# facebookresearch/DLRM-FlexFlow

Measured on AMD Instinct MI355X. Metric: dlrm_training_samples_per_sec, higher is better.
Workload: dtype f32; 1 GPU; criteo-terabyte-shape: 26 tables (rows 39884406-39043-17289-7420-20263-3-7120-1543-63-38532951-2953546-403346-10-2208-11938-155-4-976-14-39979771-25641295-39664984-585935-12972-108-36), emb_dim 128, bag 1, bot 13-512-256-128, top 3456-1024-1024-512-256-1, cat interaction, SGD lr 0.01, MSE loss; global_batch=32768, per_gpu_batch=32768, parallelism=single GPU, hipGraph-replayed step, step_graph=True

## Files before the change

dlrm_flexflow_amd/host/ffmodel.h:

```cpp
#pragma once

#include <cstddef>
#include <cstdint>
#include <condition_variable>
#include <deque>
#include <functional>
#include <map>
#include <mutex>
#include <thread>
#include <string>
#include <vector>

#include "../../include/ff_hip.h"
#include "../../include/ff_hip_bf16.h"
#include "../../include/ff_hip_ctr.h"
#include "../../include/ff_hip_lr.h"
#include "../../include/ff_hip_cross.h"
#include "../../include/ff_hip_adagrad.h"
#include "../../include/ff_hip_rowwise.h"
#include "../../include/ff_hip_fold.h"
#include "ffcomm.h"

enum ActiMode { AC_MODE_NONE = 10, AC_MODE_RELU = 11, AC_MODE_SIGMOID = 12, AC_MODE_TANH = 13, AC_MODE_GELU = 14 };
enum AggrMode { AGGR_MODE_NONE = 20, AGGR_MODE_SUM = 21, AGGR_MODE_AVG = 22 };
// ... 69 lines not shown
  bool deterministic;
  bool fp32_split_bf16x3;
  bool allow_tensor_op_math_conversion;
  bool bf16_convert_twins;
  bool bf16_exact_small_backward;
  bool bf16_twins, force_async_launch;
  bool capture_exchange;
  bool pad_linear_k;
  bool sparse_embedding_optimizer;
  int early_sort;
  bool dx_colsum;
  bool dx_scatter;
  bool fuse_pair;
  int  bucket_allreduce;
  bool direct_allreduce;
  int64_t allreduce_bucket_floats;
  int64_t big_dw_min_weights;
  int  big_dw_chunks;
  int  trace_mode;
  bool fold_small_tables;
  int64_t fold_max_rows;
  bool fold_dw;
  bool fold_dx;
  bool mlp_chain;
  int64_t mlp_chain_max_batch;
  int64_t mlp_chain_fwd_max_batch;
  int64_t mlp_chain_fwd_min_batch;
  int64_t mlp_chain_max_weights;
  bool attach_events;
  bool timing_events;
  int driver_loss;
  int eval_batches;
  int synthetic_labels;
  bool eval_only;
  int data_randomize;
  bool fuse_loss;
  int64_t replicate_embedding_rows;
  int64_t row_shard_rows;
  bool async_launch;
  bool parallel_dw;
  bool force_exchange;
  DataType embedding_dtype;
  int embedding_rounding;
  int64_t lr_warmup_steps, lr_decay_start_step, lr_num_decay_steps;
  bool device_lr;
  bool host_lr_schedule;
// ... 160 lines not shown
  virtual void backward(const FFModel&) = 0;
  virtual void create_weights(FFModel&) {}
  virtual void create_output_and_partition(FFModel&) = 0;
  virtual void print_layer(const FFModel&) const;
  OperatorType op_type;
  char name[MAX_OPNAME];
  Tensor inputs[MAX_NUM_INPUTS];
  Tensor outputs[1];
  Parameter weights[2];
  int numInputs, numWeights, numOutputs;
  int layer_index;
  bool profiling;
};

class Linear : public Op {
 public:
  Linear(FFModel& model, const Tensor& input, int out_dim, ActiMode activation, bool use_bias, const Op* shared_op,
         Initializer* kernel_initializer, Initializer* bias_initializer, const char* name);
  void create_weights(FFModel& model) override;
  void create_output_and_partition(FFModel& model) override;
  void forward(const FFModel&) override;
  void backward(const FFModel&) override;
  void backward_part(const FFModel&, int part);
  void backward_dw_rows(const FFModel&, int row0, int nrows);
  int in_channels, out_channels;
  int in_padded;
  ActiMode activation;
  bool use_bias;
  bool discard_input_grad;
  bool dx_overwrite;
  ffh_col_dest* dx_map;
  class Concat* dx_map_concat;
  Linear* pair_upper;
  mutable bool fwd_done_by_pair;
  Linear* pair_lower;
  int backward_pair(const FFModel&);
  bool dx_mask_by_x, dy_premasked;
  Linear* colsum_lower;
  bool db_from_upper;
  std::vector<Linear*> chain_fwd;
  mutable bool fwd_done_by_chain;
  void* out_twin = nullptr;
  bool bwd_exact = false;
  void* dx_twin = nullptr;
  bool dx_twin_registered = false;
  bool dx_image = false;
// ... 206 lines not shown
  int  big_dw_chunks_now() const;
  mutable int64_t n_bucket_allreduces = 0;
  int64_t n_fused_loss_calls = 0;
  mutable int64_t n_chain_fwd_calls = 0, n_chain_bwd_calls = 0;
  bool mlp_chain_usable(int64_t rows, bool fwd) const;
  int run_chain_fwd(const Linear* lowest) const;
  int run_chain_bwd(Linear* top);
  mutable bool mlp_grads_clean;
  LaunchWorker *dw_worker, *side_worker;
  std::vector<ffh_event> layer_events;
  bool use_workers() const { return dw_worker != nullptr && capturing_trace < 0; }
  ffh_event ev_fork, ev_join, ev_grad_ready, ev_update_done;
  int rank, world_size;
  bool exchange;
  int64_t local_batch;
  bool compiled;

  void* dmalloc(size_t bytes) const;
  void check(int rc, const char* what) const;

  std::vector<Embedding*> embeddings;
  void embedding_group_forward(ffh_stream s, ffh_ctx* on_ctx = nullptr) const;
  void replicated_embedding_grads() const;
  void embedding_group_update(ffh_stream s, ffh_ctx* on_ctx = nullptr) const;
  void embedding_kernels_only(bool fwd, ffh_stream s, const std::vector<const int64_t*>* idx_override = nullptr) const;
  mutable bool probe_events_on = false;
  static constexpr int kProbeEvents = 30;
  mutable ffh_event probe_ev[kProbeEvents] = {};
  void probe_record(int which, ffh_stream s, ffh_ctx* cx) const;
  uint64_t* bf16_counter = nullptr;
  ffh_bf16_rounding bf16_rounding() const;
  uint64_t read_bf16_counter() const;
  void advance_bf16_counter(ffh_stream s, ffh_ctx* cx) const;
  size_t bf16_tables_per_launch() const;
  enum LrRoute { kLrOff = 0, kLrHost = 1, kLrDevice = 2 };
  int lr_route = kLrOff;
  std::string lr_route_why;
  double lr_base = 0.0;
  int64_t lr_host_steps = 0;
  ffh_lr_state* lr_block[2] = {nullptr, nullptr};
  void lr_choose_route();
  void lr_allocate();
  void lr_host_set(int64_t k);
  void advance_lr(int which, ffh_stream s, ffh_ctx* cx) const;
  double current_lr();
  int64_t lr_steps();
  std::string lr_schedule_line() const;
// ... 32 lines not shown
    Linear* layer = nullptr;
    std::vector<Embedding*> tables;
    std::vector<ffh_fold_group> groups;
    std::vector<ffh_emb_table> gather;
    std::vector<ffh_fold_seg> keep;
    float* P = nullptr;
    float* S = nullptr;
    std::vector<Embedding*> dw_tables;
    std::vector<ffh_emb_table> dw_sum;
    std::vector<ffh_fold_group> dw_groups;
    std::vector<int32_t> dw_kept;
    float* G = nullptr;
    ffh_ctx* sum_ctx = nullptr;
    void* sum_ws = nullptr;
    bool dx = false;
  } fold;
  bool fold_dx_table(const Embedding* e) const;
  void fold_table_update(ffh_stream s, ffh_ctx* cx) const;
  ffh_event ev_fold_w_read = nullptr;
  mutable bool fold_w_read_recorded = false;
  mutable ffh_event fold_dx_event = nullptr;
  ffh_event ev_fold_e_read = nullptr;
  mutable bool fold_e_read_recorded = false;
  void fold_weight_gradient(const Linear* li, float* dbp, ffh_stream dws) const;
  ffh_event ev_fold_w = nullptr;
  ffh_event ev_fold_done = nullptr;
  mutable bool fold_w_recorded = false, fold_on_side = false;
  void plan_fold();
  void plan_fold_dw(FoldRoute& r);
  void plan_fold_dx(FoldRoute& r);
  void fold_products_and_sum(ffh_stream s, ffh_ctx* cx) const;
  void fold_linear_forward(const Linear* li) const;
  int z_reader_layer;
  ffh_event ev_z_free;
  mutable bool z_free_recorded;
  mutable bool grad_ready_attached;

  float *mlp_weights, *mlp_grads;  size_t mlp_count;
  char* act_slab;
  char* act_grad_slab;  size_t act_grad_bytes;
  void* workspace;  size_t workspace_bytes;
  void* repl_workspace;  size_t repl_workspace_bytes;
  ffh_perf_metrics* d_perf;
  float* d_bce_sum;
  ffh_ctr_eval* d_eval;
  bool want_eval;
  bool evaluating;
// ... 24 lines not shown
```

dlrm_flexflow_amd/host/ffmodel_c.cc:

```cpp
#include <cstring>
#include "ffmodel_c.h"
#include <string>

#include <chrono>

#include <cstdio>
#include <cstdlib>
#include <vector>

#include "backend.h"
#include "dlrm.h"
#include "ffmodel.h"

namespace {
FFConfig* C(flexflow_config_t h) { return (FFConfig*)h.impl; }
FFModel* M(flexflow_model_t h) { return (FFModel*)h.impl; }
Tensor* T(flexflow_tensor_t h) { return (Tensor*)h.impl; }
Initializer* I(flexflow_initializer_t h) { return (Initializer*)h.impl; }
DLRMApp* A(flexflow_dlrm_t h) { return (DLRMApp*)h.impl; }
flexflow_tensor_t wrap(const Tensor& t) { flexflow_tensor_t h; h.impl = new Tensor(t); return h; }
std::vector<int> dims_vec(const int* dims, int n) { return std::vector<int>(dims, dims + n); }
}

extern "C" {
// ... 132 lines not shown
void flexflow_model_set_trace_mode(flexflow_model_t m, int mode) { M(m)->config.trace_mode = mode; }
int flexflow_model_trace_replays(flexflow_model_t m, int trace_id) { return M(m)->trace_replays(trace_id) ? 1 : 0; }
int64_t flexflow_model_get_counter(flexflow_model_t m, const char* name) {
  const std::string n(name ? name : "");
  if (n == "mlp_chain_fwd_calls") return M(m)->n_chain_fwd_calls;
  if (n == "mlp_chain_bwd_calls") return M(m)->n_chain_bwd_calls;
  if (n == "fused_loss_calls") return M(m)->n_fused_loss_calls;
  if (n == "allreduce_bucket_calls") return M(m)->n_bucket_allreduces;
  if (n == "allreduce_buckets") return (int64_t)M(m)->grad_buckets.size();
  if (n.rfind("allreduce_bucket_floats_", 0) == 0) {
    const size_t k = (size_t)atoi(n.c_str() + 24);
    return k < M(m)->grad_buckets.size() ? (int64_t)M(m)->grad_buckets[k].count : -1;
  }
  if (n == "allreduce_bucket_channel_own") return M(m)->config.comm.bucket_channel_own;
  if (n == "direct_allreduces") return M(m)->n_direct_allreduces;
  if (n == "bf16_updates") return (int64_t)M(m)->read_bf16_counter();
  if (n == "early_sorts") return M(m)->n_early_sorts;
  if (n == "lr_steps") return M(m)->lr_steps();
  if (n == "lr_route") return M(m)->lr_route;
  if (n == "graph_replays") return M(m)->n_graph_replays;
  if (n == "folded_tables") return (int64_t)M(m)->fold.tables.size();
  if (n == "folded_dw_tables") return (int64_t)M(m)->fold.dw_tables.size();
  if (n == "folded_dx_tables") return (int64_t)(M(m)->fold.dx ? M(m)->fold.dw_tables.size() : 0);
  if (n == "tensor_op_exact_backward_layers") {
    int64_t k = 0;
    for (Op* op : M(m)->layers) if (op->op_type == OP_LINEAR && static_cast<Linear*>(op)->bwd_exact) k++;
    return k;
  }
  return -1;
}

int flexflow_model_save_checkpoint(flexflow_model_t m, const char* dir, int64_t epochs_done) { M(m)->save_checkpoint(dir ? dir : "", epochs_done); return 0; }
int flexflow_model_load_checkpoint(flexflow_model_t m, const char* dir, int64_t* epochs_done) {
  const FFModel::CheckpointInfo info = M(m)->load_checkpoint(dir ? dir : "");
  if (epochs_done) *epochs_done = info.epochs_done;
  return 0;
}
uint64_t flexflow_model_state_digest(flexflow_model_t m) { return M(m)->state_digest(); }
uint64_t flexflow_state_digest_host(const void* base, int64_t rows, int64_t row_bytes, int64_t ld_bytes, uint64_t seed, uint64_t index_base) {
  return ffh_state_digest_host(base, rows, row_bytes, ld_bytes, seed, index_base);
}
uint64_t flexflow_digest_record_seed(uint64_t ordinal) { return ffh_digest_record_seed(ordinal); }

int flexflow_tensor_get_num_dims(flexflow_tensor_t t) { return T(t)->numDim; }
void flexflow_tensor_get_dims(flexflow_tensor_t t, int* dims) { for (int i = 0; i < T(t)->numDim; i++) dims[i] = T(t)->adim[T(t)->numDim - 1 - i]; }
int64_t flexflow_tensor_get_local_rows(flexflow_tensor_t t) { return T(t)->impl ? T(t)->impl->rows_local : 0; }
// ... 175 lines not shown
```

dlrm_flexflow_amd/host/model.cc:

```cpp
#include "ffmodel.h"
#include "model_internal.h"


LaunchWorker::LaunchWorker(const KernelApi* _api, int _device) : api(_api), device(_device), wctx(nullptr), stop(false), busy(false) {
  th = std::thread([this] { run(); });
  drain();
}
LaunchWorker::~LaunchWorker() {
  {
    std::lock_guard<std::mutex> lk(mu);
    stop = true;
  }
  cv.notify_all();
  if (th.joinable()) th.join();
  if (wctx) api->ffh_ctx_destroy(wctx);
}
void LaunchWorker::run() {
  {
    ffh_ctx* c = nullptr;
    if (api->ffh_ctx_create(&c, device) != FFH_OK) die("launch worker: ffh_ctx_create(device %d) failed", device);
    std::lock_guard<std::mutex> lk(mu);
    wctx = c;
  }
  cv_idle.notify_all();
// ... 324 lines not shown
  for (ffh_event e : layer_events) api->ffh_event_destroy(ctx, e);
  for (auto& kv : graphs) api->ffh_graph_destroy(ctx, kv.second);
  for (TensorImpl* t : tensor_impls) {
    if (t->ptr && !t->alias && t->bytes) api->ffh_free(ctx, t->ptr);
    delete t;
  }
  for (void* p : {w_twin, act_twin, grad_twin, (void*)ar_scratch}) if (p) api->ffh_free(ctx, p);
  for (void* p : {(void*)mlp_weights, (void*)mlp_grads, (void*)act_slab, (void*)act_grad_slab, workspace, repl_workspace, (void*)d_perf, (void*)d_bce_sum, (void*)d_eval, (void*)digest_acc, (void*)xsend,
                  (void*)xrecv, (void*)gsend, (void*)grecv})
    if (p) api->ffh_free(ctx, p);
  for (Embedding* e : embeddings)
    for (void* p : {(void*)e->local_idx, (void*)e->partial, (void*)e->gfull, (void*)e->opt_state[0], (void*)e->opt_state[1]})
      if (p) api->ffh_free(ctx, p);
  for (Op* op : layers)
    if (op->op_type == OP_LINEAR && static_cast<Linear*>(op)->dx_map) api->ffh_free(ctx, static_cast<Linear*>(op)->dx_map);
  api->ffh_event_destroy(ctx, ev_fork); api->ffh_event_destroy(ctx, ev_join);
  api->ffh_event_destroy(ctx, ev_grad_ready); api->ffh_event_destroy(ctx, ev_update_done);
  api->ffh_event_destroy(ctx, ev_dw_done);
  api->ffh_event_destroy(ctx, ev_z_free);
  if (ev_fold_w) api->ffh_event_destroy(ctx, ev_fold_w);
  if (ev_fold_done) api->ffh_event_destroy(ctx, ev_fold_done);
  if (ev_fold_e_read) api->ffh_event_destroy(ctx, ev_fold_e_read);
  if (ev_fold_w_read) api->ffh_event_destroy(ctx, ev_fold_w_read);
  for (void* p : {(void*)fold.P, (void*)fold.S, (void*)fold.G, fold.sum_ws}) if (p) api->ffh_free(ctx, p);
  if (fold.sum_ctx) api->ffh_ctx_destroy(fold.sum_ctx);
  for (auto& kv : trace_tune) for (ffh_event& e : kv.second.ev) if (e) { api->ffh_event_destroy(ctx, e); e = nullptr; }
  for (ffh_event& e : probe_ev) if (e) { api->ffh_event_destroy(ctx, e); e = nullptr; }
  api->ffh_stream_destroy(ctx, stream); api->ffh_stream_destroy(ctx, side_stream); api->ffh_stream_destroy(ctx, dw_stream); api->ffh_stream_destroy(ctx, ar_stream);
  for (GradBucket& b : grad_buckets) { api->ffh_event_destroy(ctx, b.ready); api->ffh_event_destroy(ctx, b.ready_dw); api->ffh_event_destroy(ctx, b.done); }
  api->ffh_ctx_destroy(ctx);
  for (Op* op : layers) delete op;
  for (Initializer* i : owned_initializers) delete i;
  for (Tensor* t : input_tensors) delete t;
}

void FFModel::check(int rc, const char* what) const {
  if (rc != FFH_OK) die("%s failed (%d): %s", what, rc, api->ffh_last_error_string(ctx));
}

void* FFModel::dmalloc(size_t bytes) const {
  void* p = nullptr;
  int rc = api->ffh_malloc(ctx, &p, bytes);
  if (rc != FFH_OK || !p) die("device allocation of %zu bytes failed: %s", bytes, api->ffh_last_error_string(ctx));
  return p;
}

// ... 125 lines not shown
  else if (out_twin) ff.check(ff.api->ffh_convert_f32_to_bf16(ff.ctx, out_twin, (const float*)y.impl->ptr, b * (int64_t)y.impl->ld, ff.stream), name);
}
int Linear::backward_pair(const FFModel& ff) {
  Linear* lo = pair_lower;
  const Tensor &xu = inputs[0], &yu = outputs[0], &xl = lo->inputs[0];
  const int64_t b = local_rows(yu, &ff);
  const int flags_u = dy_premasked ? FFH_LINEAR_DY_PREMASKED : 0;
  const int flags_l = (lo->dx_overwrite ? FFH_LINEAR_DX_OVERWRITE : 0) | (lo->dx_mask_by_x ? FFH_LINEAR_DX_MASK_BY_X : 0);
  const int rc = ff.api->ffh_linear_pair_bwd(
      ff.ctx, (const float*)xu.impl->ptr, xu.impl->ld, (const float*)yu.impl->ptr, yu.impl->ld, yu.impl->grad, yu.impl->grad_ld,
      (const float*)weights[0].impl->ptr, weights[0].impl->grad, (use_bias && !db_from_upper) ? weights[1].impl->grad : nullptr, in_channels, out_channels,
      (int)activation, flags_u, (const float*)xl.impl->ptr, xl.impl->ld, xl.impl->grad, xl.impl->grad_ld, xu.impl->grad, xu.impl->grad_ld,
      (const float*)lo->weights[0].impl->ptr, lo->in_channels, (int)lo->activation, flags_l, b, ff.stream);
  if (rc != FFH_OK) return rc;
  db_from_upper = false;
  ff.check(ff.api->ffh_linear_bwd_ex(ff.ctx, (const float*)xl.impl->ptr, xl.impl->ld, nullptr, xl.impl->grad_ld, (const float*)xu.impl->ptr, xu.impl->ld,
                                     xu.impl->grad, xu.impl->grad_ld, (const float*)lo->weights[0].impl->ptr, lo->weights[0].impl->grad,
                                     lo->use_bias ? lo->weights[1].impl->grad : nullptr, lo->in_channels, lo->out_channels, b, (int)lo->activation,
                                     FFH_LINEAR_ONLY_DW | FFH_LINEAR_DY_PREMASKED, ff.stream, nullptr), lo->name);
  return FFH_OK;
}
void Linear::backward(const FFModel& ff) { backward_part(ff, 0); }

void Linear::backward_part(const FFModel& ff, int part) {
  if (activation == AC_MODE_GELU) die("%s: GELU has no backward (forward / inference only, as in the reference)", name);
  const Tensor& x = inputs[0];
  const Tensor& y = outputs[0];
  const int64_t b = local_rows(y, &ff);
  float* dx = discard_input_grad ? nullptr : x.impl->grad;
  const double macs = (double)in_channels * out_channels * (double)b;
  const bool fork = ff.config.parallel_dw && macs >= 1.0e8;
  const int flags = (dx_overwrite ? FFH_LINEAR_DX_OVERWRITE : 0) | (dx_mask_by_x ? FFH_LINEAR_DX_MASK_BY_X : 0) | (dy_premasked ? FFH_LINEAR_DY_PREMASKED : 0);
  const float *xp = (const float*)x.impl->ptr, *yp = (const float*)y.impl->ptr, *wp = (const float*)weights[0].impl->ptr;
  float *dyp = y.impl->grad, *dwp = weights[0].impl->grad, *dbp = (use_bias && !db_from_upper) ? weights[1].impl->grad : nullptr;
  const int64_t ldx = x.impl->ld, lddx = x.impl->grad_ld, ldy = y.impl->ld, lddy = y.impl->grad_ld;
  if (part != 1) db_from_upper = false;
  struct ColsumScope {
    const FFModel& ff; Linear* lo;
    ColsumScope(const FFModel& f, Linear* l, bool produces_dx) : ff(f), lo(produces_dx ? l : nullptr) {
      if (lo) ff.check(ff.api->ffh_linear_bwd_set_dx_colsum(ff.ctx, lo->weights[1].impl->grad, lo->out_channels), "dx colsum");
    }
    ~ColsumScope() { if (lo) lo->db_from_upper = ff.api->ffh_linear_dx_colsum_used(ff.ctx) != 0; }
  } colsum_scope(ff, colsum_lower, dx != nullptr && (part == 0 || part == 1) && !ff.use_workers() && !ff.config.profiling && !(ff.fold.layer == this && ff.fold.dx));
  auto image_dx = [&] {
    if (dx_image && dx) ff.check(ff.api->ffh_convert_f32_to_bf16x3(ff.ctx, dx, b, in_channels, lddx, ff.stream), name);
    if (bwd_exact && dx && dx_twin) ff.check(ff.api->ffh_convert_f32_to_bf16(ff.ctx, dx_twin, dx, b * (int64_t)in_channels, ff.stream), name);
  };
  struct ExactScope {
    const FFModel& ff; bool on;
    ExactScope(const FFModel& f, bool o) : ff(f), on(o) { if (on) ff.check(ff.api->ffh_ctx_set_math_mode(ff.ctx, FFH_MATH_DEFAULT), "math mode"); }
    ~ExactScope() { if (on) ff.check(ff.api->ffh_ctx_set_math_mode(ff.ctx, FFH_MATH_TENSOR_OP_BF16), "math mode"); }
  } exact_scope(ff, bwd_exact && !ff.use_workers());
  if (part == 1) {
    ff.check(ff.api->ffh_linear_bwd_ex(ff.ctx, xp, ldx, dx, lddx, yp, ldy, dyp, lddy, wp, dwp, dbp, in_padded, out_channels, b, (int)activation,
// ... 17 lines not shown
    ff.check(api->ffh_linear_bwd_ex(ff.ctx, xp, ldx, dx, lddx, yp, ldy, dyp, lddy, wp, dwp, dbp, in, out, b, act, flags | FFH_LINEAR_ONLY_DX, ff.stream, nullptr), name);
    if (sig) { ff.check(api->ffh_event_record(ff.ctx, ev, ff.stream), "event"); ff.dw_worker->post(dw_call); }
    ff.dw_forked = true;
    return;
  }
  ffh_stream dws = ff.dw_stream;
  if (part == 0 && ff.fold.layer == this && !ff.fold.dw_tables.empty()) {
    if (fork) {
      ffh_event ev = ff.layer_events[layer_index];
      ff.check(ff.api->ffh_event_record(ff.ctx, ev, ff.stream), "event");
      ff.check(ff.api->ffh_stream_wait_event(ff.ctx, dws, ev), "event");
    }
    if (dx && ff.fold.dx) {
      ffh_event ev = ff.fold_dx_event;
      ff.fold_dx_event = nullptr;
      ff.check(ff.api->fold->ffh_fold_linear_bwd_dx(ff.ctx, xp, ldx, dx, lddx, dyp, lddy, wp, in_padded, out_channels, b,
                                                    flags & (FFH_LINEAR_DX_OVERWRITE | FFH_LINEAR_DX_MASK_BY_X), ff.fold.dw_kept.data(), (int)ff.fold.dw_kept.size(),
                                                    nullptr, ev, ff.stream), name);
    } else if (dx) {
      ff.check(ff.api->ffh_linear_bwd_ex(ff.ctx, xp, ldx, dx, lddx, yp, ldy, dyp, lddy, wp, dwp, dbp, in_padded, out_channels, b, (int)activation,
                                         flags | FFH_LINEAR_ONLY_DX, ff.stream, nullptr), name);
      image_dx();
    }
    ff.fold_weight_gradient(this, dbp, fork ? dws : ff.stream);
    if (fork) { ff.dw_forked = true; ff.dw1_used = true; ff.dw_stream_used_directly = true; }
    return;
  }
  ff.check(ff.api->ffh_linear_bwd_ex(ff.ctx, xp, ldx, dx, lddx, yp, ldy, dyp, lddy, wp, dwp, dbp, in_padded, out_channels, b, (int)activation,
                                     flags, ff.stream, fork ? dws : nullptr), name);
  image_dx();
  if (fork) { ff.dw_forked = true; ff.dw1_used = true; }
}

void Linear::backward_dw_rows(const FFModel& ff, int row0, int nrows) {
  const Tensor& x = inputs[0];
  const Tensor& y = outputs[0];
  const int64_t b = local_rows(y, &ff);
  const float *xp = (const float*)x.impl->ptr, *yp = (const float*)y.impl->ptr + row0;
  float *dyp = y.impl->grad + row0, *dwp = weights[0].impl->grad + (size_t)row0 * (size_t)weights[0].impl->ld;
  const float* wp = (const float*)weights[0].impl->ptr + (size_t)row0 * (size_t)weights[0].impl->ld;
  float* dbp = (use_bias && !db_from_upper) ? weights[1].impl->grad + row0 : nullptr;
  const int flags = FFH_LINEAR_ONLY_DW | FFH_LINEAR_DY_PREMASKED;
  ff.check(ff.api->ffh_linear_bwd_ex(ff.ctx, xp, x.impl->ld, nullptr, x.impl->grad_ld, yp, y.impl->ld, dyp, y.impl->grad_ld, wp, dwp, dbp, in_padded, nrows, b,
                                     (int)activation, flags, ff.dw_stream, nullptr), name);
  ff.dw_forked = true;
  ff.dw1_used = true;
  ff.dw_stream_used_directly = true;
// ... 546 lines not shown
```

dlrm_flexflow_amd/host/model_allocate.cc:

```cpp
#include "model_internal.h"

int FFModel::tables_of_rank(int r) const {
  int n = 0;
  for (const Embedding* e : embeddings) n += e->owner_rank == r;
  return n;
}

int FFModel::next_seed() {
  return (int)(ffh_hash(config.seed * 0x9E3779B97F4A7C15ULL + 0x5EED, seed_counter++) & 0x7fffffffULL);
}

bool FFModel::fused_embedding_update() const {
  if (config.dense_embedding_update) return false;
  const SGDOptimizer* sgd = dynamic_cast<const SGDOptimizer*>(optimizer);
  if (sgd && sgd->momentum == 0.0 && sgd->weight_decay == 0.0) return true;
  const AdagradOptimizer* adagrad = dynamic_cast<const AdagradOptimizer*>(optimizer);
  if (adagrad && adagrad->weight_decay == 0.0) return true;
  return config.sparse_embedding_optimizer && (sgd || adagrad || dynamic_cast<const AdamOptimizer*>(optimizer));
}

bool FFModel::sparse_rule(ffh_sparse_opt& o) const {
  memset(&o, 0, sizeof o);
  if (const SGDOptimizer* sgd = dynamic_cast<const SGDOptimizer*>(optimizer)) {
    o.lr = (float)sgd->lr;
// ... 935 lines not shown
  const Embedding* e0 = r.tables[pick[0]];
  const int L = (int)e0->inputs[0].adim[0];
  r.G = (float*)dmalloc((size_t)grows * out * 4);
  const size_t ws_bytes = api->ffh_embedding_bwd_workspace_bytes((int)pick.size(), L, out, local_batch) + 256;
  r.sum_ws = dmalloc(ws_bytes);
  if (api->ffh_ctx_create(&r.sum_ctx, config.device) != FFH_OK || !r.sum_ctx) die("fold: ffh_ctx_create(device %d) failed", config.device);
  check(api->ffh_ctx_set_workspace(r.sum_ctx, r.sum_ws, ws_bytes), "set workspace");
  int64_t grow = 0;
  for (size_t k : pick) {
    Embedding* e = r.tables[k];
    float* g = r.G + (size_t)grow * out;
    r.dw_tables.push_back(e);
    r.dw_groups.push_back(ffh_fold_group{(const float*)e->weights[0].impl->ptr, (int64_t)e->out_channels, r.groups[k].col0, g, (int64_t)e->num_entries});
    ffh_emb_table t;
    t.idx = (const int64_t*)e->inputs[0].impl->ptr;
    t.weight = g;
    t.num_entries = e->num_entries;
    t.io = y.impl->grad;
    t.ld = y.impl->grad_ld;
    r.dw_sum.push_back(t);
    grow += e->num_entries;
  }
  if (!ev_fold_e_read) check((config.timing_events ? api->ffh_event_create : api->ffh_event_create_sync)(ctx, &ev_fold_e_read), "event create");
  plan_fold_dx(r);
}

void FFModel::plan_fold_dx(FoldRoute& r) {
  Linear* li = r.layer;
  if (!config.fold_dx || r.dw_tables.empty() || !api->fold->ffh_fold_linear_bwd_dx || !api->fold->ffh_fold_linear_bwd_dx_plan || !api->fold->ffh_fold_table_update) return;
  ffh_sparse_opt rule;
  if (!fused_embedding_update() || sparse_rule(rule) || !config.overlap_embedding || use_workers()) return;
  if (lr_route == kLrDevice && !api->fold->ffh_fold_table_update_lr) return;
  if (li->discard_input_grad || li->colsum_lower || li->inputs[0].impl->grad == nullptr) return;
  const Embedding* e0 = r.dw_tables[0];
  if (e0->out_channels % 64) return;
  const Tensor &x = li->inputs[0], &y = li->outputs[0];
  const int flags = (li->dx_overwrite ? FFH_LINEAR_DX_OVERWRITE : 0) | (li->dx_mask_by_x ? FFH_LINEAR_DX_MASK_BY_X : 0);
  const int plan = api->fold->ffh_fold_linear_bwd_dx_plan(ctx, (const float*)x.impl->ptr, x.impl->ld, x.impl->grad, x.impl->grad_ld, y.impl->grad, y.impl->grad_ld,
                                                          (const float*)li->weights[0].impl->ptr, li->in_padded, li->out_channels, local_rows(y, this), flags,
                                                          r.dw_kept.data(), (int)r.dw_kept.size(), nullptr);
  if (plan != 1) return;
  r.dx = true;
  if (!ev_fold_w_read) check((config.timing_events ? api->ffh_event_create : api->ffh_event_create_sync)(ctx, &ev_fold_w_read), "event create");
}

void FFModel::init_layers() {
// ... 9 lines not shown
```

dlrm_flexflow_amd/host/model_exchange.cc:

```cpp
#include "model_internal.h"

void launch_shard_groups(const FFModel* ff, ShardLaunch what, ffh_stream s, ffh_ctx* cx, const std::vector<const int64_t*>* idx_override, bool all_tables) {
  const bool fwd = what == kGather;
  ffh_sparse_opt rule;
  const bool ruled = (what == kFusedUpdate || what == kApplyOnly) && ff->sparse_rule(rule);
  const ffh_lr_state* lrb = ff->lr_route == FFModel::kLrDevice ? ff->lr_block[1] : nullptr;
  const KernelApiLr* lra = ff->api->lr;
  const int L = ff->embeddings[0]->inputs[0].adim[0];
  const int aggr = (int)ff->embeddings[0]->aggr;
  struct Group { std::vector<ffh_emb_table> t; std::vector<ffh_emb_table_bf16> t16; std::vector<ffh_emb_state> st; };
  std::map<std::pair<int, bool>, Group> groups;
  size_t owned_i = 0;
  for (const FFModel::EmbShard& sh : ff->shards) {
    if (sh.owner != ff->rank) continue;
    const Embedding* e = sh.e;
    ffh_emb_table t;
    t.idx = (const int64_t*)e->inputs[0].impl->ptr;
    if (idx_override && owned_i < idx_override->size()) t.idx = (*idx_override)[owned_i];
    owned_i++;
    if (!fwd && !all_tables && ff->fold_dx_table(e)) continue;
    t.weight = (float*)e->weights[0].impl->ptr;
    t.num_entries = e->num_entries;
    if (!ff->exchange) {
      t.io = fwd ? (float*)e->outputs[0].impl->ptr : e->outputs[0].impl->grad;
// ... 162 lines not shown
void FFModel::replicated_embedding_grads() const {
  if (!repl_workspace) return;
  std::vector<ffh_emb_table> tabs;
  const int L = embeddings[0]->inputs[0].adim[0], D = embeddings[0]->out_channels;
  for (const Embedding* e : embeddings) {
    if (!e->replicated) continue;
    ffh_emb_table t;
    t.idx = (const int64_t*)e->inputs[0].impl->ptr + (int64_t)rank * local_batch * L;
    t.weight = e->weights[0].impl->grad;
    t.num_entries = e->num_entries;
    t.io = e->outputs[0].impl->grad;
    t.ld = e->outputs[0].impl->grad_ld;
    tabs.push_back(t);
  }
  check(api->ffh_ctx_set_workspace(ctx, repl_workspace, repl_workspace_bytes), "set workspace");
  for (size_t b = 0; b < tabs.size(); b += FFH_MAX_TABLES) {
    const int n = (int)std::min<size_t>(FFH_MAX_TABLES, tabs.size() - b);
    check(api->ffh_embedding_bwd_sgd_fused_multi(ctx, tabs.data() + b, n, L, D, local_batch, (int)embeddings[0]->aggr, -1.0f, stream),
          "embedding gradient (data-parallel tables)");
  }
  check(api->ffh_ctx_set_workspace(ctx, workspace, workspace_bytes), "set workspace");
}

void FFModel::embedding_group_update(ffh_stream s, ffh_ctx* on_ctx) const {
  if (embeddings.empty()) return;
  if (exchange) {
    probe_record(6, s, on_ctx ? on_ctx : ctx);
    if (!shards.empty() && config.comm.alltoall_f32(config.comm.user, gsend, fwd_recv_counts.data(), grecv, fwd_send_counts.data(), s) != 0)
      die("alltoall (embedding backward) failed");
    probe_record(7, s, on_ctx ? on_ctx : ctx);
    bwd_alltoall_issued = true;
  }
  launch_shard_groups(this, emb_sorted_early ? kApplyOnly : kFusedUpdate, s, on_ctx ? on_ctx : ctx);
  emb_sorted_early = false;
  ffh_ctx* cx = on_ctx ? on_ctx : ctx;
  ffh_sparse_opt rule;
  const bool ruled = sparse_rule(rule);
  for (const Embedding* e : embeddings) {
    if (!e->row_sharded) continue;
    const int L = e->inputs[0].adim[0], D = e->out_channels;
    if (config.comm.allgather_f32(config.comm.user, e->outputs[0].impl->grad, e->gfull, local_batch * D, s) != 0)
      die("all-gather (row-sharded embedding backward) failed");
    float* w = (float*)e->weights[0].impl->ptr;
    if (ruled) {
      const ffh_emb_table t{e->local_idx, w, e->gfull, e->rows_local + 1, D};
      const ffh_emb_state st{e->opt_state[0], e->opt_state[1]};
      check(api->ffh_embedding_bwd_opt_fused_multi(cx, &t, &st, 1, L, D, config.batchSize, (int)e->aggr, &rule, s), e->name);
    } else {
      check(api->ffh_embedding_bwd_sgd_fused(cx, e->local_idx, e->gfull, w, L, D, config.batchSize, e->rows_local + 1, D, (int)e->aggr, rule.lr, s), e->name);
    }
    check(api->ffh_zero(cx, w + e->rows_local * (int64_t)D, (size_t)D * 4, s), "zero row");
  }
  advance_bf16_counter(s, cx);
  advance_lr(1, s, cx);
}

void FFModel::embedding_dense_update() const {
  if (embeddings.empty()) return;
  const int L = embeddings[0]->inputs[0].adim[0];
  const int aggr = (int)embeddings[0]->aggr;
  if (exchange) {
    if (!shards.empty() && config.comm.alltoall_f32(config.comm.user, gsend, fwd_recv_counts.data(), grecv, fwd_send_counts.data(), stream) != 0)
      die("alltoall (embedding backward) failed");
    for (const EmbShard& sh : shards) {
      if (sh.owner != rank) continue;
      const Embedding* e = sh.e;
      check(api->ffh_embedding_bwd_dense(ctx, (const int64_t*)e->inputs[0].impl->ptr, grecv + sh.off, e->weights[0].impl->grad, L, sh.cols,
                                         config.batchSize, e->num_entries, rank_width[rank], aggr, stream), e->name);
    }
    for (const Embedding* e : embeddings) {
      if (!e->row_sharded) continue;
      const int D = e->out_channels;
      if (config.comm.allgather_f32(config.comm.user, e->outputs[0].impl->grad, e->gfull, local_batch * D, stream) != 0)
        die("all-gather (row-sharded embedding backward) failed");
      check(api->ffh_embedding_bwd_dense(ctx, e->local_idx, e->gfull, e->weights[0].impl->grad, L, D, config.batchSize, e->rows_local + 1, D, aggr, stream), e->name);
    }
  }
// ... 76 lines not shown
```

dlrm_flexflow_amd/host/model_flags.cc:

```cpp
#include "model_internal.h"

FFConfig::FFConfig() {
  epochs = 1;
  batchSize = 64;
  printFreq = 10;
  numNodes = 1;
  cpusPerNode = 0;
  workersPerNode = 0;
  learningRate = 0.01f;
  weightDecay = 0.0001f;
  workSpaceSize = (size_t)1 << 30;
  syntheticInput = false;
  profiling = false;
  perform_fusion = false;
  computationMode = COMP_MODE_TRAINING;
  device = 0;
  seed = 0;
  enable_graph = true;
  overlap_embedding = true;
  dense_embedding_update = false;
  force_exchange = false;
  parallel_dw = true;
  async_launch = false;
  column_shard_rows = 0;
  row_shard_rows = 0;
  replicate_embedding_rows = 0;
  fuse_loss = true;
  driver_loss = LOSS_MEAN_SQUARED_ERROR_AVG_REDUCE;
  eval_batches = 0;
  eval_only = false;
  synthetic_labels = 0;
  data_randomize = 0;
  timing_events = false;
  attach_events = true;
  fuse_pair = true;
  mlp_chain = true;
  fold_small_tables = true;
  fold_max_rows = 7420;
  fold_dw = true;
  fold_dx = true;
  trace_mode = -1;
  bucket_allreduce = -1;
  allreduce_bucket_floats = 1 << 20;
  direct_allreduce = false;
  big_dw_chunks = 0;
  big_dw_min_weights = 2 << 20;
  mlp_chain_max_batch = 8192;
  mlp_chain_fwd_max_batch = 4096;
  mlp_chain_fwd_min_batch = 4096;
  mlp_chain_max_weights = 200000;
  dx_scatter = true;
  dx_colsum = true;
  early_sort = -1;
  pad_linear_k = true;
  capture_exchange = false;
  bf16_twins = true;
  bf16_convert_twins = true;
  bf16_exact_small_backward = true;
  force_async_launch = false;
  sparse_embedding_optimizer = false;
  allow_tensor_op_math_conversion = false;
  fp32_split_bf16x3 = false;
  deterministic = false;
// ... 66 lines not shown
    if (is("--eval-batches")) { eval_batches = atoi(next()); if (eval_batches < 0) die("--eval-batches %d: must be >= 0", eval_batches); continue; }
    if (is("--eval-only")) { eval_only = true; continue; }
    if (is("--synthetic-labels")) {
      const char* v = next();
      if (!strcmp(v, "bernoulli")) synthetic_labels = 0;
      else if (!strcmp(v, "logistic")) synthetic_labels = 1;
      else die("--synthetic-labels %s: 'bernoulli' or 'logistic'", v);
      continue;
    }
    if (is("--data-randomize")) {
      const char* v = next();
      if (!strcmp(v, "none")) data_randomize = 0;
      else if (!strcmp(v, "total")) data_randomize = 1;
      else die("--data-randomize %s: 'none' or 'total'", v);
      continue;
    }
    if (is("--timing-events")) { timing_events = true; continue; }
    if (is("--no-attach-event")) { attach_events = false; continue; }
    if (is("--no-fused-pair")) { fuse_pair = false; continue; }
    if (is("--no-mlp-chain")) { mlp_chain = false; continue; }
    if (is("--no-fold-small-tables")) { fold_small_tables = false; continue; }
    if (is("--no-fold-dw")) { fold_dw = false; continue; }
    if (is("--no-fold-dx")) { fold_dx = false; continue; }
    if (is("--fold-max-rows")) { fold_max_rows = atoll(next()); continue; }
    if (is("--always-replay")) { trace_mode = 1; continue; }
    if (is("--adaptive-replay")) { trace_mode = 0; continue; }
    if (is("--bucket-allreduce")) { bucket_allreduce = 1; continue; }
    if (is("--no-bucket-allreduce")) { bucket_allreduce = 0; continue; }
    if (is("--allreduce-bucket-floats")) { allreduce_bucket_floats = atoll(next()); continue; }
    if (is("--direct-allreduce")) { direct_allreduce = true; continue; }
    if (is("--big-dw-chunks")) { big_dw_chunks = atoi(next()); continue; }
    if (is("--big-dw-min-weights")) { big_dw_min_weights = atoll(next()); continue; }
    if (is("--mlp-chain-max-batch")) { mlp_chain_max_batch = atoll(next()); continue; }
    if (is("--mlp-chain-fwd-min-batch")) { mlp_chain_fwd_min_batch = atoll(next()); continue; }
    if (is("--mlp-chain-fwd-max-batch")) { mlp_chain_fwd_max_batch = atoll(next()); continue; }
    if (is("--mlp-chain-max-weights")) { mlp_chain_max_weights = atoll(next()); continue; }
    if (is("--no-dx-scatter")) { dx_scatter = false; continue; }
    if (is("--no-dx-colsum")) { dx_colsum = false; continue; }
    if (is("--no-early-sort")) { early_sort = 0; continue; }
    if (is("--early-sort")) { early_sort = 1; continue; }
    if (is("--no-pad-linear-k")) { pad_linear_k = false; continue; }
    if (is("--capture-exchange")) { capture_exchange = true; continue; }
    if (is("--no-bf16-exact-small-backward")) { bf16_exact_small_backward = false; continue; }
    if (is("--no-bf16-convert-twins")) { bf16_convert_twins = false; continue; }
    if (is("--no-bf16-twins")) { bf16_twins = false; continue; }
    if (is("--force-async-launch")) { force_async_launch = true; continue; }
// ... 33 lines not shown
```

dlrm_flexflow_amd/host/model_step.cc:

```cpp
#include "model_internal.h"

void FFModel::reset_metrics() {
  if (replaying_trace >= 0) return;
  check(api->ffh_zero(ctx, d_perf, sizeof(ffh_perf_metrics), stream), "reset_metrics");
  if (d_bce_sum) check(api->ffh_zero(ctx, d_bce_sum, sizeof(float), stream), "reset_metrics");
}

void FFModel::refresh_weight_twin() const {
  if (!w_twin || !w_twin_dirty) return;
  if (config.fp32_split_bf16x3 && !config.allow_tensor_op_math_conversion) check(api->ffh_convert_f32_to_bf16x3(ctx, mlp_weights, 1, (int64_t)mlp_count, (int64_t)mlp_count, stream), "weight image");
  else check(api->ffh_convert_f32_to_bf16(ctx, w_twin, mlp_weights, (int64_t)mlp_count, stream), "weight twin");
  w_twin_dirty = false;
}
int64_t FFModel::weight_mirror_stale_bytes() {
  if (!w_twin) return -1;
  if (w_twin_dirty) return -2;
  sync();
  const bool x3 = config.fp32_split_bf16x3 && !config.allow_tensor_op_math_conversion;
  const size_t bytes = x3 ? FFH_BF16X3_IMAGE_BYTES((size_t)mlp_count * 4) : (size_t)mlp_count * 2;
  std::vector<char> kept(bytes), fresh(bytes);
  check(api->ffh_memcpy_d2h(ctx, kept.data(), w_twin, bytes, stream), "weight mirror d2h");
  w_twin_dirty = true;
  refresh_weight_twin();
  check(api->ffh_memcpy_d2h(ctx, fresh.data(), w_twin, bytes, stream), "weight mirror d2h");
// ... 74 lines not shown
      check(api->ffh_stream_wait_event(ctx, side_stream, ev_fold_w), "fold: weights ready");
      fold_products_and_sum(side_stream, ctx);
      check(api->ffh_event_record(ctx, ev_fold_done, side_stream), "fold: sum ready");
      fold_on_side = true;
    }
    if (early_sort_possible(1)) {
      launch_shard_groups(this, kSortOnly, side_stream, ctx);
      emb_sorted_early = true;
    }
  }
  emb_forward_issued = true;
  emb_forward_joined = false;
}

void FFModel::fold_products_and_sum(ffh_stream s, ffh_ctx* cx) const {
  const Linear* li = fold.layer;
  const Embedding* e0 = fold.tables[0];
  check(api->fold->ffh_fold_product(cx, fold.groups.data(), (int)fold.groups.size(), (const float*)li->weights[0].impl->ptr, li->in_padded, e0->out_channels,
                                    li->out_channels, s), "fold_product");
  check(api->fold->ffh_fold_gather_add(cx, fold.gather.data(), (int)fold.gather.size(), e0->inputs[0].adim[0], li->out_channels, local_batch, FFH_AGGR_MODE_SUM,
                                       fold.S, li->out_channels, s), "fold_gather_add");
}

void FFModel::fold_weight_gradient(const Linear* li, float* dbp, ffh_stream dws) const {
  const Tensor &x = li->inputs[0], &y = li->outputs[0];
  const Embedding* e0 = fold.dw_tables[0];
  const int64_t b = local_rows(y, this);
  const int out = li->out_channels, ng = (int)fold.dw_groups.size();
  if (api->fold->ffh_fold_segment_sum(fold.sum_ctx, fold.dw_sum.data(), ng, e0->inputs[0].adim[0], out, b, dws) != FFH_OK)
    die("%s: fold_segment_sum failed: %s", li->name, api->ffh_last_error_string(fold.sum_ctx));
  check(api->fold->ffh_fold_dw_product(ctx, fold.dw_groups.data(), ng, li->weights[0].impl->grad, li->in_padded, e0->out_channels, out, dws), "fold_dw_product");
  check(api->ffh_event_record(ctx, ev_fold_e_read, dws), "fold: table rows read");
  fold_e_read_recorded = true;
  check(api->fold->ffh_fold_linear_bwd_dw(ctx, (const float*)x.impl->ptr, x.impl->ld, y.impl->grad, y.impl->grad_ld, li->weights[0].impl->grad, dbp, li->in_padded, out, b,
                                          fold.dw_kept.data(), (int)fold.dw_kept.size(), dws), li->name);
}

void FFModel::fold_table_update(ffh_stream s, ffh_ctx* cx) const {
  const Linear* li = fold.layer;
  const Embedding* e0 = fold.dw_tables[0];
  const int ng = (int)fold.dw_groups.size();
  const float* w = (const float*)li->weights[0].impl->ptr;
  if (lr_route == kLrDevice) {
    check(api->fold->ffh_fold_table_update_lr(cx, fold.dw_groups.data(), ng, w, li->in_padded, e0->out_channels, li->out_channels, lr_block[1], s), "fold_table_update_lr");
  } else {
    ffh_sparse_opt rule;
    sparse_rule(rule);
    check(api->fold->ffh_fold_table_update(cx, fold.dw_groups.data(), ng, w, li->in_padded, e0->out_channels, li->out_channels, rule.lr, s), "fold_table_update");
  }
}
bool FFModel::fold_dx_table(const Embedding* e) const {
  if (!fold.dx) return false;
  for (const Embedding* t : fold.dw_tables) if (t == e) return true;
  return false;
}

void FFModel::fold_linear_forward(const Linear* li) const {
  if (fold_on_side) check(api->ffh_stream_wait_event(ctx, stream, ev_fold_done), "fold: sum ready");
  else fold_products_and_sum(stream, ctx);
// ... 2 lines not shown
  check(api->fold->ffh_fold_linear_fwd(ctx, (const float*)x.impl->ptr, x.impl->ld, (float*)y.impl->ptr, y.impl->ld, (const float*)li->weights[0].impl->ptr,
                                       li->use_bias ? (const float*)li->weights[1].impl->ptr : nullptr, li->in_padded, li->out_channels, local_rows(y, this),
                                       (int)li->activation, fold.keep.data(), (int)fold.keep.size(), fold.S, li->out_channels, stream), li->name);
}

void FFModel::join_embedding_forward() const {
  if (side_worker) side_worker->drain();
  probe_record(10, stream, ctx);
  check(api->ffh_stream_wait_event(ctx, stream, ev_join), "join");
  probe_record(11, stream, ctx);
  emb_forward_joined = true;
}

void FFModel::issue_embedding_update_on_side_stream() const {
  if (use_workers()) {
    const FFModel* self = this;
    side_worker->post([self](ffh_ctx* wc) {
      self->check(self->api->ffh_stream_wait_event(wc, self->side_stream, self->ev_grad_ready), "event");
      self->embedding_group_update(self->side_stream, wc);
      self->check(self->api->ffh_event_record(wc, self->ev_update_done, self->side_stream), "event");
    });
  } else {
    check(api->ffh_stream_wait_event(ctx, side_stream, ev_grad_ready), "event");
    if (fold_e_read_recorded) check(api->ffh_stream_wait_event(ctx, side_stream, ev_fold_e_read), "fold: table rows read");
    probe_record(2, side_stream, ctx);
    if (fold.dx) {
      if (!fold_e_read_recorded) die("fold: the dx-folded tables' update without this step's segmented sum");
      fold_table_update(side_stream, ctx);
      check(api->ffh_event_record(ctx, ev_fold_w_read, side_stream), "fold: weights read");
      fold_w_read_recorded = true;
    }
    embedding_group_update(side_stream);
    probe_record(3, side_stream, ctx);
    check(api->ffh_event_record(ctx, ev_update_done, side_stream), "event");
  }
}

void FFModel::order_input_writes_behind_update() const {
  if (embeddings.empty() || !config.overlap_embedding || !fused_embedding_update()) return;
  if (side_worker) side_worker->drain();
  check(api->ffh_stream_wait_event(ctx, stream, ev_update_done), "inputs behind the table update");
}

void FFModel::zero_gradients() {
  if (replaying_trace >= 0) return;
  if (need_zero_act_grads) check(api->ffh_zero(ctx, act_grad_slab, act_grad_bytes, stream), "zero_gradients");
// ... 7 lines not shown
    for (Embedding* e : embeddings)
      if (e->held_here(rank) && !e->replicated)
        check(api->ffh_zero(ctx, e->weights[0].impl->grad, e->weights[0].impl->bytes + (e->row_sharded ? (size_t)e->out_channels * 4 : 0), stream), "zero_gradients");
}

void FFModel::compute_metrics() {
  if (replaying_trace >= 0) return;
  const Tensor& fin = layers.back()->outputs[0];
  check(api->ffh_metrics_update(ctx, (const float*)fin.impl->ptr, (const float*)label_tensor.impl->ptr, d_perf,
                                local_rows(fin, this), fin.adim[0], metrics_flags, stream), "compute_metrics");
}

void FFModel::backward(int _seq_length) {
  if (replaying_trace >= 0) return;
  seq_length = _seq_length;
  if (config.computationMode != COMP_MODE_TRAINING) die("backward() in inference mode");
  const Tensor& fin = layers.back()->outputs[0];
  const bool bce = loss_type == LOSS_BINARY_CROSSENTROPY;
  const float scale = (bce || loss_type == LOSS_MEAN_SQUARED_ERROR_AVG_REDUCE) ? 1.0f / (float)fin.adim[fin.numDim - 1] : 1.0f;
  if (fin.impl->grad_ld != fin.adim[0] || fin.impl->ld != fin.adim[0]) die("final layer output must be contiguous");
  dw_forked = false;
  fold_e_read_recorded = false;
  fold_w_read_recorded = false;
  fold_dx_event = nullptr;
  opt_next_done = false;
  int first = (int)layers.size() - 1;
  emb_update_pending = false;
  mlp_grads_clean = false;
  Linear* last = (config.fuse_loss && !config.profiling) ? dynamic_cast<Linear*>(layers.back()) : nullptr;
  int rc = FFH_ERR_UNSUPPORTED;
  if (last) {
    const Tensor& x = last->inputs[0];
    const int flags = (last->dx_overwrite ? FFH_LINEAR_DX_OVERWRITE : 0) | (last->dx_mask_by_x ? FFH_LINEAR_DX_MASK_BY_X : 0);
    if (bce)
      rc = api->ctr->ffh_linear_bwd_bce(ctx, (const float*)x.impl->ptr, x.impl->ld, last->discard_input_grad ? nullptr : x.impl->grad, x.impl->grad_ld,
                                        (const float*)fin.impl->ptr, fin.impl->ld, fin.impl->grad, fin.impl->grad_ld,
                                        (const float*)last->weights[0].impl->ptr, last->weights[0].impl->grad,
                                        last->use_bias ? last->weights[1].impl->grad : nullptr, last->in_channels, last->out_channels,
                                        local_rows(fin, this), (int)last->activation, flags, (const float*)label_tensor.impl->ptr, scale, d_perf,
                                        d_bce_sum, metrics_flags, stream);
    else
    rc = api->ffh_linear_bwd_mse(ctx, (const float*)x.impl->ptr, x.impl->ld, last->discard_input_grad ? nullptr : x.impl->grad, x.impl->grad_ld,
                                 (const float*)fin.impl->ptr, fin.impl->ld, fin.impl->grad, fin.impl->grad_ld,
                                 (const float*)last->weights[0].impl->ptr, last->weights[0].impl->grad,
                                 last->use_bias ? last->weights[1].impl->grad : nullptr, last->in_channels, last->out_channels,
                                 local_rows(fin, this), (int)last->activation, flags, (const float*)label_tensor.impl->ptr, scale, d_perf,
// ... 65 lines not shown
      const int crc = run_chain_bwd(up);
      if (crc == FFH_OK) {
        if (grad_attach_layer > l - n && grad_attach_layer < l && !grad_ready_attached) {
          check(api->ffh_event_record(ctx, ev_grad_ready, stream), "event");
          grad_ready_attached = true;
        }
        for (int k = 0; k < n; k++) mark_z_free(l - k);
        l -= n - 1;
        continue;
      }
      if (crc != FFH_ERR_UNSUPPORTED) check(crc, up->name);
      up->chain_bwd.clear();
    }
    if (up && up->pair_lower && !use_workers() && l != grad_attach_layer && l >= 1 && layers[l - 1] == up->pair_lower) {
      const int prc = up->backward_pair(*this);
      if (prc == FFH_OK) { l--; continue; }
      if (prc != FFH_ERR_UNSUPPORTED) check(prc, up->name);
      up->pair_lower = nullptr;
    }
    if (up && dw_chunks > 1 && l == big_dw_layer) { chunked_big_backward(up, l); mark_z_free(l); continue; }
    layers[l]->backward(*this);
    mark_z_free(l);
  }
  if (emb_update_pending) {
    issue_embedding_update_on_side_stream();
    emb_update_pending = false;
  }
  if (bucketed_now()) { bwd_alltoall_issued = true; issue_grad_buckets(-1); }
}

void FFModel::update() {
  n_update_calls++;
  if (replaying_trace >= 0) return;
  optimizer->next();
  opt_next_done = true;
  SGDOptimizer* sgd = dynamic_cast<SGDOptimizer*>(optimizer);
  AdamOptimizer* adam = dynamic_cast<AdamOptimizer*>(optimizer);
  AdagradOptimizer* adagrad = dynamic_cast<AdagradOptimizer*>(optimizer);
  if (!sgd && !adam && !adagrad) die("update(): unknown optimizer");
  if (side_worker) side_worker->drain();
  if (dw_forked && !dw_worker && !api->ffh_second_stream_used(ctx, 1) && !dw_stream_used_directly) { dw_forked = false; dw1_used = false; }
  dw_stream_used_directly = false;
  if (dw_forked) {
    if (dw_worker) { dw_worker->drain(); dw1_used = true; }
    if (dw1_used) {
      check(api->ffh_event_record(ctx, ev_dw_done, dw_stream), "join dw");
      check(api->ffh_stream_wait_event(ctx, stream, ev_dw_done), "join dw");
    }
    if (config.overlap_embedding && !embeddings.empty() && !use_workers()) {
      if (z_free_recorded) check(api->ffh_stream_wait_event(ctx, side_stream, ev_z_free), "join dw (embedding stream)");
      else {
        if (dw1_used) check(api->ffh_stream_wait_event(ctx, side_stream, ev_dw_done), "join dw (embedding stream)");
      }
    }
    dw1_used = false;
    dw_forked = false;
  }
  if (exchange && mlp_count) {
    bool any_issued = false;
    for (const GradBucket& b : grad_buckets) any_issued = any_issued || b.issued;
    if (any_issued) {
      for (const GradBucket& b : grad_buckets) if (!b.issued) die("update(): a gradient bucket was not issued");
      probe_record(12, stream, ctx);
      for (const GradBucket& b : grad_buckets) if (!b.inline_issued) check(api->ffh_stream_wait_event(ctx, stream, b.done), "join all-reduce bucket");
      probe_record(13, stream, ctx);
      probe_record(8, stream, ctx);
      for (auto& r : grad_rest)
        if (allreduce_grads(mlp_grads + r.first, (int64_t)r.second, stream, false) != 0) die("allreduce failed");
      probe_record(9, stream, ctx);
    } else {
      probe_record(8, stream, ctx);
      if (allreduce_grads(mlp_grads, (int64_t)mlp_count, stream, false) != 0) die("allreduce failed");
      probe_record(9, stream, ctx);
    }
  }
  if (fold_w_read_recorded) { check(api->ffh_stream_wait_event(ctx, stream, ev_fold_w_read), "fold: weights read"); fold_w_read_recorded = false; }
  const size_t opt_count = mlp_count;
  const ffh_lr_state* lrb = lr_route == kLrDevice ? lr_block[0] : nullptr;
  if (adam) {
    if (mlp_count && lrb) {
// ... 315 lines not shown
```

Measured before the change: 5.302 million samples/s.

## Reschedule folded-table dW GEMM onto compute stream and update folded tables early

For the layer that consumes the folded small embedding tables, the kept-column weight-gradient GEMM is deferred to the end of backward and run on the main compute stream, instead of sitting behind the fold segmented-sum on the dW stream. An event records when that GEMM has read the layer input so the embedding stream can wait on it. The side-stream embedding update is also reordered to run the regular table update first, then the folded-table update once the segmented sum has read the rows. The learning-rate advance is moved to after both updates. Both behaviours are on by default, with flags to opt out. The aim is better overlap between streams, at the cost of extra cross-stream dependencies and a possible ordering hazard on the shared input buffer.

```diff
diff --git a/dlrm_flexflow_amd/host/ffmodel.h b/dlrm_flexflow_amd/host/ffmodel.h
--- a/dlrm_flexflow_amd/host/ffmodel.h
+++ b/dlrm_flexflow_amd/host/ffmodel.h
@@ -115,6 +115,8 @@
   int64_t fold_max_rows;
   bool fold_dw;
   bool fold_dx;
+  bool fold_dw_behind_sum;
+  bool fold_update_behind_products;
   bool mlp_chain;
   int64_t mlp_chain_max_batch;
   int64_t mlp_chain_fwd_max_batch;
@@ -321,6 +323,7 @@
   void forward(const FFModel&) override;
   void backward(const FFModel&) override;
   void backward_part(const FFModel&, int part);
+  bool forks_dw(const FFModel&) const;
   void backward_dw_rows(const FFModel&, int row0, int nrows);
   int in_channels, out_channels;
   int in_padded;
@@ -573,7 +576,7 @@
   std::vector<Embedding*> embeddings;
   void embedding_group_forward(ffh_stream s, ffh_ctx* on_ctx = nullptr) const;
   void replicated_embedding_grads() const;
-  void embedding_group_update(ffh_stream s, ffh_ctx* on_ctx = nullptr) const;
+  void embedding_group_update(ffh_stream s, ffh_ctx* on_ctx = nullptr, bool advance_rate = true) const;
   void embedding_kernels_only(bool fwd, ffh_stream s, const std::vector<const int64_t*>* idx_override = nullptr) const;
   mutable bool probe_events_on = false;
   static constexpr int kProbeEvents = 30;
@@ -652,7 +655,17 @@
   mutable ffh_event fold_dx_event = nullptr;
   ffh_event ev_fold_e_read = nullptr;
   mutable bool fold_e_read_recorded = false;
-  void fold_weight_gradient(const Linear* li, float* dbp, ffh_stream dws) const;
+  void fold_weight_gradient(const Linear* li, float* dbp, ffh_stream dws, ffh_stream gemm_stream) const;
+  void fold_kept_dw_gemm(const Linear* li, float* dbp, ffh_stream s, bool off_dw_stream) const;
+  mutable bool fold_dw_defer = false;
+  mutable const Linear* fold_dw_pending = nullptr;
+  mutable float* fold_dw_pending_db = nullptr;
+  bool fold_schedule_route() const;
+  bool fold_dw_on_compute() const;
+  bool fold_update_early() const;
+  ffh_event ev_fold_x_read = nullptr;
+  mutable bool fold_x_read_recorded = false;
+  mutable int64_t n_fold_dw_on_compute = 0, n_fold_update_early = 0;
   ffh_event ev_fold_w = nullptr;
   ffh_event ev_fold_done = nullptr;
   mutable bool fold_w_recorded = false, fold_on_side = false;
diff --git a/dlrm_flexflow_amd/host/ffmodel_c.cc b/dlrm_flexflow_amd/host/ffmodel_c.cc
--- a/dlrm_flexflow_amd/host/ffmodel_c.cc
+++ b/dlrm_flexflow_amd/host/ffmodel_c.cc
@@ -178,6 +178,8 @@
   if (n == "folded_tables") return (int64_t)M(m)->fold.tables.size();
   if (n == "folded_dw_tables") return (int64_t)M(m)->fold.dw_tables.size();
   if (n == "folded_dx_tables") return (int64_t)(M(m)->fold.dx ? M(m)->fold.dw_tables.size() : 0);
+  if (n == "fold_dw_on_compute_steps") return M(m)->n_fold_dw_on_compute;
+  if (n == "fold_update_early_steps") return M(m)->n_fold_update_early;
   if (n == "tensor_op_exact_backward_layers") {
     int64_t k = 0;
     for (Op* op : M(m)->layers) if (op->op_type == OP_LINEAR && static_cast<Linear*>(op)->bwd_exact) k++;
diff --git a/dlrm_flexflow_amd/host/model.cc b/dlrm_flexflow_amd/host/model.cc
--- a/dlrm_flexflow_amd/host/model.cc
+++ b/dlrm_flexflow_amd/host/model.cc
@@ -370,6 +370,7 @@
   if (ev_fold_done) api->ffh_event_destroy(ctx, ev_fold_done);
   if (ev_fold_e_read) api->ffh_event_destroy(ctx, ev_fold_e_read);
   if (ev_fold_w_read) api->ffh_event_destroy(ctx, ev_fold_w_read);
+  if (ev_fold_x_read) api->ffh_event_destroy(ctx, ev_fold_x_read);
   for (void* p : {(void*)fold.P, (void*)fold.S, (void*)fold.G, fold.sum_ws}) if (p) api->ffh_free(ctx, p);
   if (fold.sum_ctx) api->ffh_ctx_destroy(fold.sum_ctx);
   for (auto& kv : trace_tune) for (ffh_event& e : kv.second.ev) if (e) { api->ffh_event_destroy(ctx, e); e = nullptr; }
@@ -541,14 +542,18 @@
 }
 void Linear::backward(const FFModel& ff) { backward_part(ff, 0); }
 
+bool Linear::forks_dw(const FFModel& ff) const {
+  const double macs = (double)in_channels * out_channels * (double)local_rows(outputs[0], &ff);
+  return ff.config.parallel_dw && macs >= 1.0e8;
+}
+
 void Linear::backward_part(const FFModel& ff, int part) {
   if (activation == AC_MODE_GELU) die("%s: GELU has no backward (forward / inference only, as in the reference)", name);
   const Tensor& x = inputs[0];
   const Tensor& y = outputs[0];
   const int64_t b = local_rows(y, &ff);
   float* dx = discard_input_grad ? nullptr : x.impl->grad;
-  const double macs = (double)in_channels * out_channels * (double)b;
-  const bool fork = ff.config.parallel_dw && macs >= 1.0e8;
+  const bool fork = forks_dw(ff);
   const int flags = (dx_overwrite ? FFH_LINEAR_DX_OVERWRITE : 0) | (dx_mask_by_x ? FFH_LINEAR_DX_MASK_BY_X : 0) | (dy_premasked ? FFH_LINEAR_DY_PREMASKED : 0);
   const float *xp = (const float*)x.impl->ptr, *yp = (const float*)y.impl->ptr, *wp = (const float*)weights[0].impl->ptr;
   float *dyp = y.impl->grad, *dwp = weights[0].impl->grad, *dbp = (use_bias && !db_from_upper) ? weights[1].impl->grad : nullptr;
@@ -612,7 +617,7 @@
                                          flags | FFH_LINEAR_ONLY_DX, ff.stream, nullptr), name);
       image_dx();
     }
-    ff.fold_weight_gradient(this, dbp, fork ? dws : ff.stream);
+    ff.fold_weight_gradient(this, dbp, fork ? dws : ff.stream, fork && !ff.fold_dw_on_compute() ? dws : ff.stream);
     if (fork) { ff.dw_forked = true; ff.dw1_used = true; ff.dw_stream_used_directly = true; }
     return;
   }
diff --git a/dlrm_flexflow_amd/host/model_allocate.cc b/dlrm_flexflow_amd/host/model_allocate.cc
--- a/dlrm_flexflow_amd/host/model_allocate.cc
+++ b/dlrm_flexflow_amd/host/model_allocate.cc
@@ -981,6 +981,7 @@
     grow += e->num_entries;
   }
   if (!ev_fold_e_read) check((config.timing_events ? api->ffh_event_create : api->ffh_event_create_sync)(ctx, &ev_fold_e_read), "event create");
+  if (!ev_fold_x_read) check((config.timing_events ? api->ffh_event_create : api->ffh_event_create_sync)(ctx, &ev_fold_x_read), "event create");
   plan_fold_dx(r);
 }
 
diff --git a/dlrm_flexflow_amd/host/model_exchange.cc b/dlrm_flexflow_amd/host/model_exchange.cc
--- a/dlrm_flexflow_amd/host/model_exchange.cc
+++ b/dlrm_flexflow_amd/host/model_exchange.cc
@@ -208,7 +208,7 @@
   check(api->ffh_ctx_set_workspace(ctx, workspace, workspace_bytes), "set workspace");
 }
 
-void FFModel::embedding_group_update(ffh_stream s, ffh_ctx* on_ctx) const {
+void FFModel::embedding_group_update(ffh_stream s, ffh_ctx* on_ctx, bool advance_rate) const {
   if (embeddings.empty()) return;
   if (exchange) {
     probe_record(6, s, on_ctx ? on_ctx : ctx);
@@ -238,7 +238,7 @@
     check(api->ffh_zero(cx, w + e->rows_local * (int64_t)D, (size_t)D * 4, s), "zero row");
   }
   advance_bf16_counter(s, cx);
-  advance_lr(1, s, cx);
+  if (advance_rate) advance_lr(1, s, cx);
 }
 
 void FFModel::embedding_dense_update() const {
diff --git a/dlrm_flexflow_amd/host/model_flags.cc b/dlrm_flexflow_amd/host/model_flags.cc
--- a/dlrm_flexflow_amd/host/model_flags.cc
+++ b/dlrm_flexflow_amd/host/model_flags.cc
@@ -39,6 +39,8 @@
   fold_max_rows = 7420;
   fold_dw = true;
   fold_dx = true;
+  fold_dw_behind_sum = false;
+  fold_update_behind_products = false;
   trace_mode = -1;
   bucket_allreduce = -1;
   allreduce_bucket_floats = 1 << 20;
@@ -151,6 +153,8 @@
     if (is("--no-fold-small-tables")) { fold_small_tables = false; continue; }
     if (is("--no-fold-dw")) { fold_dw = false; continue; }
     if (is("--no-fold-dx")) { fold_dx = false; continue; }
+    if (is("--fold-dw-behind-sum")) { fold_dw_behind_sum = true; continue; }
+    if (is("--fold-update-behind-products")) { fold_update_behind_products = true; continue; }
     if (is("--fold-max-rows")) { fold_max_rows = atoll(next()); continue; }
     if (is("--always-replay")) { trace_mode = 1; continue; }
     if (is("--adaptive-replay")) { trace_mode = 0; continue; }
diff --git a/dlrm_flexflow_amd/host/model_step.cc b/dlrm_flexflow_amd/host/model_step.cc
--- a/dlrm_flexflow_amd/host/model_step.cc
+++ b/dlrm_flexflow_amd/host/model_step.cc
@@ -120,8 +120,8 @@
                                        fold.S, li->out_channels, s), "fold_gather_add");
 }
 
-void FFModel::fold_weight_gradient(const Linear* li, float* dbp, ffh_stream dws) const {
-  const Tensor &x = li->inputs[0], &y = li->outputs[0];
+void FFModel::fold_weight_gradient(const Linear* li, float* dbp, ffh_stream dws, ffh_stream gemm_stream) const {
+  const Tensor& y = li->outputs[0];
   const Embedding* e0 = fold.dw_tables[0];
   const int64_t b = local_rows(y, this);
   const int out = li->out_channels, ng = (int)fold.dw_groups.size();
@@ -130,9 +130,24 @@
   check(api->fold->ffh_fold_dw_product(ctx, fold.dw_groups.data(), ng, li->weights[0].impl->grad, li->in_padded, e0->out_channels, out, dws), "fold_dw_product");
   check(api->ffh_event_record(ctx, ev_fold_e_read, dws), "fold: table rows read");
   fold_e_read_recorded = true;
-  check(api->fold->ffh_fold_linear_bwd_dw(ctx, (const float*)x.impl->ptr, x.impl->ld, y.impl->grad, y.impl->grad_ld, li->weights[0].impl->grad, dbp, li->in_padded, out, b,
-                                          fold.dw_kept.data(), (int)fold.dw_kept.size(), dws), li->name);
-}
+  if (gemm_stream != dws && fold_dw_defer) { fold_dw_pending = li; fold_dw_pending_db = dbp; return; }
+  fold_kept_dw_gemm(li, dbp, gemm_stream, gemm_stream != dws);
+}
+void FFModel::fold_kept_dw_gemm(const Linear* li, float* dbp, ffh_stream s, bool off_dw_stream) const {
+  const Tensor &x = li->inputs[0], &y = li->outputs[0];
+  check(api->fold->ffh_fold_linear_bwd_dw(ctx, (const float*)x.impl->ptr, x.impl->ld, y.impl->grad, y.impl->grad_ld, li->weights[0].impl->grad, dbp, li->in_padded, li->out_channels,
+                                          local_rows(y, this), fold.dw_kept.data(), (int)fold.dw_kept.size(), s), li->name);
+  if (off_dw_stream) {
+    check(api->ffh_event_record(ctx, ev_fold_x_read, s), "fold: layer input read");
+    fold_x_read_recorded = true;
+    n_fold_dw_on_compute++;
+  }
+}
+bool FFModel::fold_schedule_route() const {
+  return fold.layer && !fold.dw_tables.empty() && fold.layer->forks_dw(*this) && config.overlap_embedding && !use_workers() && !config.profiling;
+}
+bool FFModel::fold_dw_on_compute() const { return fold_schedule_route() && !config.fold_dw_behind_sum; }
+bool FFModel::fold_update_early() const { return fold_schedule_route() && fold.dx && !config.fold_update_behind_products; }
 
 void FFModel::fold_table_update(ffh_stream s, ffh_ctx* cx) const {
   const Linear* li = fold.layer;
@@ -181,6 +196,20 @@
     });
   } else {
     check(api->ffh_stream_wait_event(ctx, side_stream, ev_grad_ready), "event");
+    if (fold_update_early()) {
+      if (!fold_e_read_recorded) die("fold: the dx-folded tables' update without this step's segmented sum");
+      probe_record(2, side_stream, ctx);
+      embedding_group_update(side_stream, nullptr, false);
+      check(api->ffh_stream_wait_event(ctx, side_stream, ev_fold_e_read), "fold: table rows read");
+      fold_table_update(side_stream, ctx);
+      check(api->ffh_event_record(ctx, ev_fold_w_read, side_stream), "fold: weights read");
+      fold_w_read_recorded = true;
+      advance_lr(1, side_stream, ctx);
+      probe_record(3, side_stream, ctx);
+      check(api->ffh_event_record(ctx, ev_update_done, side_stream), "event");
+      n_fold_update_early++;
+      return;
+    }
     if (fold_e_read_recorded) check(api->ffh_stream_wait_event(ctx, side_stream, ev_fold_e_read), "fold: table rows read");
     probe_record(2, side_stream, ctx);
     if (fold.dx) {
@@ -234,6 +263,9 @@
   dw_forked = false;
   fold_e_read_recorded = false;
   fold_w_read_recorded = false;
+  fold_x_read_recorded = false;
+  fold_dw_pending = nullptr;
+  fold_dw_defer = true;
   fold_dx_event = nullptr;
   opt_next_done = false;
   int first = (int)layers.size() - 1;
@@ -345,6 +377,11 @@
     layers[l]->backward(*this);
     mark_z_free(l);
   }
+  fold_dw_defer = false;
+  if (fold_dw_pending) {
+    fold_kept_dw_gemm(fold_dw_pending, fold_dw_pending_db, stream, true);
+    fold_dw_pending = nullptr;
+  }
   if (emb_update_pending) {
     issue_embedding_update_on_side_stream();
     emb_update_pending = false;
@@ -379,6 +416,7 @@
     dw1_used = false;
     dw_forked = false;
   }
+  if (fold_x_read_recorded) { check(api->ffh_stream_wait_event(ctx, side_stream, ev_fold_x_read), "fold: layer input read (embedding stream)"); fold_x_read_recorded = false; }
   if (exchange && mlp_count) {
     bool any_issued = false;
     for (const GradBucket& b : grad_buckets) any_issued = any_issued || b.issued;
```

Result: faster. 5.355 million samples/s, median of 6 (+1.0%).
